# jcfaracco/xpysom-dask

Hardware: AMD Instinct MI355X
Metric: samples/sec/epoch (higher is better)
Workload: dtype f16

## Files before the change

### xpysom_dask_amd/_lib.py

```python
import ctypes as C
import importlib.util
import os

HERE = os.path.dirname(os.path.abspath(__file__))
LIB_PATH = os.environ.get("SOM_LIB_PATH") or os.path.join(HERE, "libsomhip.so")

SOM_DIST = {"euclidean": 0, "euclidean_no_opt": 1, "cosine": 2, "manhattan": 3, "manhattan_no_opt": 3,
            "norm_p": 4, "norm_p_no_opt": 5}
SOM_NEIGH = {"gaussian": 0, "mexican_hat": 1, "bubble": 2, "triangle": 3}
SOM_PREC = {"f32": 0, "bf16": 1, "f16": 3, "exact": 5}
SOM_TOPO = {"rectangular": 0, "hexagonal": 1}
SOM_BMU_ACTIVATION, SOM_BMU_QUANTIZATION = 0, 1
SOM_KERNELS = {"bmu": 0, "segsum": 1, "kron": 2, "merge": 3, "prep": 4, "screen": 5}


class SomConfig(C.Structure):
    _fields_ = [("x", C.c_int32), ("y", C.c_int32), ("input_len", C.c_int32),
                ("distance", C.c_int32), ("neighborhood", C.c_int32),
                ("compact_support", C.c_int32), ("precision", C.c_int32), ("device", C.c_int32),
                ("std_coeff", C.c_double), ("stream", C.c_void_p),
                ("topology", C.c_int32), ("norm_p", C.c_int32), ("norm_p_real", C.c_double)]


_F = C.POINTER(C.c_float)
# ... 28 lines not shown
    "som_pinned_free": (C.c_int, [C.c_void_p]),
    "som_stream_begin": (C.c_int, [_H]),
    "som_stream_rows": (C.c_int, [_H, _F, C.c_int64]),
    "som_stream_end": (C.c_int, [_H, C.c_double, C.c_double, C.c_int]),
    "som_accum_device_ptr": (C.c_int, [_H, C.POINTER(C.c_void_p), C.POINTER(C.c_int64)]),
    "som_get_stream": (C.c_int, [_H, C.POINTER(C.c_void_p)]),
    "som_epoch_fetch": (C.c_int, [_H, _F, _F, _I]),
    "som_epoch_accumulate_forced": (C.c_int, [_H, _I, C.c_double, C.c_double, C.c_int]),
    "som_bmu": (C.c_int, [_H, _F, C.c_int64, C.c_int32, _I]),
    "som_bmu_device": (C.c_int, [_H, C.c_void_p, C.c_int64, C.c_int32, _I]),
    "som_bmu_top2": (C.c_int, [_H, _F, C.c_int64, _I, _I]),
    "som_bmu_top2_device": (C.c_int, [_H, C.c_void_p, C.c_int64, _I, _I]),
    "som_bmu_f64": (C.c_int, [_H, C.POINTER(C.c_double), C.c_int64, _I]),
    "som_distance_matrix": (C.c_int, [_H, _F, C.c_int64, C.c_int32, _F]),
    "som_quantization_error": (C.c_int, [_H, _F, C.c_int64, C.POINTER(C.c_double)]),
    "som_quantization_error_device": (C.c_int, [_H, C.c_void_p, C.c_int64, C.POINTER(C.c_double)]),
    "som_set_verify": (C.c_int, [_H, C.c_int32]),
    "som_verify_stats": (C.c_int, [_H, C.POINTER(C.c_int64), C.POINTER(C.c_int64)]),
    "som_debug_corrupt_operands": (C.c_int, [_H, C.c_int32]),
    "som_debug_mfma16": (C.c_int, [_H, C.c_void_p, C.c_void_p, _F, _F, C.c_int32]),
    "som_debug_stamps": (C.c_int, [_H, C.c_int64, C.c_void_p]),
    "som_debug_device_bytes": (C.c_int, [C.POINTER(C.c_int64)]),
    "som_debug_qe_stats": (C.c_int, [_H, C.POINTER(C.c_int64), C.POINTER(C.c_int64)]),
    "som_policy_eval": (C.c_int, [C.c_int32, C.POINTER(C.c_double), C.POINTER(C.c_double), C.POINTER(C.c_int32)]),
    "som_policy_replay": (C.c_int, [C.c_int32, C.POINTER(C.c_double), C.POINTER(C.c_double)]),
    "som_patch_order": (C.c_int, [C.c_int32, C.c_int32, _I]),
    "som_exact_stats": (C.c_int, [_H, C.POINTER(C.c_int64), C.POINTER(C.c_int64), C.POINTER(C.c_int64)]),
    "som_exact_top2_stats": (C.c_int, [_H, C.POINTER(C.c_int64), C.POINTER(C.c_int64)]),
    "som_exact_skip_stats": (C.c_int, [_H, C.POINTER(C.c_int64), C.POINTER(C.c_int64)]),
    "som_exact_resident_stats": (C.c_int, [_H, C.POINTER(C.c_int64), C.POINTER(C.c_int64)]),
    "som_exact_scout_stats": (C.c_int, [_H, C.POINTER(C.c_int64), C.POINTER(C.c_int64)]),
    "som_exact_refine_stats": (C.c_int, [_H, C.POINTER(C.c_int64), C.POINTER(C.c_int64)]),
    "som_exact_last_counts": (C.c_int, [_H, _I, C.c_int64]),
    "som_sync": (C.c_int, [_H]),
    "som_profile_enable": (C.c_int, [_H, C.c_int32]),
    "som_profile_get": (C.c_int, [_H, C.c_int32, C.POINTER(C.c_double), C.POINTER(C.c_int64)]),
    "som_profile_reset": (C.c_int, [_H]),
}

_lib = None


def torch_lib_file(name):
    try:
        spec = importlib.util.find_spec("torch")
    except (ImportError, ValueError):
# ... 46 lines not shown
```

### xpysom_dask_amd/csrc/bmu_bf16_k16.hpp

```cpp
#pragma once
#include "bmu_bf16.hpp"

namespace somhip {

constexpr int K16_T = 4;
constexpr int K16_STAGE_UNITS = 16 * K16_T;
constexpr int K16_SB = 4;
constexpr int K16_NW = 4;
constexpr int K16_WG_SAMPLES = K16_NW * 16 * K16_SB;

__host__ __device__ constexpr int k16_stage_bytes(int ks32) { return (K16_T * ks32 + 1) * 1024; }

template <int KS32, class EL = Bf16>
__global__ __launch_bounds__(256) void prep_w_bf16_k16_kernel(const float* __restrict__ W, int K, int D,
                                                              char* __restrict__ Wst, int n_stages,
                                                              const float* __restrict__ unit_wsq,
                                                              const float* __restrict__ scale_max2 = nullptr) {
    using E = typename EL::T;
    using bf16x8 = typename V8<E>::t;
    long id = (long)blockIdx.x * 256 + threadIdx.x;
    long total = (long)n_stages * K16_T * KS32 * 64;
    if (id >= total) return;
    int lane = id & 63;
    long t = id >> 6;
    int ks = t % KS32; t /= KS32;
    int t16 = t % K16_T;
    long stage = t / K16_T;
    long u = stage * K16_STAGE_UNITS + t16 * 16 + (lane & 15);
    int k0 = ks * 32 + (lane >> 4) * 8;
    float scale = 1.0f;
    if (unit_wsq != nullptr && u < K) { float q = unit_wsq[u]; scale = q > 0.0f ? 1.0f / __builtin_sqrtf(q) : 0.0f; }
    if (scale_max2 != nullptr) scale = ex_scale(*scale_max2);
    bf16x8 v;
#pragma unroll
    for (int j = 0; j < 8; ++j) {
        float f = (u < K && k0 + j < D) ? W[u * D + k0 + j] * scale : 0.0f;
        v[j] = cvt<E>(-f);
    }
    *(bf16x8*)(Wst + stage * k16_stage_bytes(KS32) + ((long)(t16 * KS32 + ks) * 64 + lane) * 16) = v;
}

template <int KS32, class EL = Bf16>
__global__ __launch_bounds__(256) void prep_w_exact_k16_kernel(const float* __restrict__ W, int K, int D,
                                                               char* __restrict__ Wst, int n_stages,
                                                               const float* __restrict__ scale_max2,
                                                               float* __restrict__ werr2, char* __restrict__ Wst_lo = nullptr) {
    using E = typename EL::T;
    using bf16x8 = typename V8<E>::t;
    const int lane = threadIdx.x & 63;
    const long tile = (long)blockIdx.x * 4 + (threadIdx.x >> 6);
    if (tile >= (long)n_stages * K16_T) return;
    const long stage = tile / K16_T;
    const int t16 = (int)(tile - stage * K16_T);
    const long u = stage * K16_STAGE_UNITS + t16 * 16 + (lane & 15);
    const float scale = ex_scale(*scale_max2);
    float er = 0.0f;
#pragma unroll
    for (int ks = 0; ks < KS32; ++ks) {
        const int k0 = ks * 32 + (lane >> 4) * 8;
        bf16x8 v, vl;
#pragma unroll
        for (int j = 0; j < 8; ++j) {
            const float f = (u < K && k0 + j < D) ? W[u * D + k0 + j] * scale : 0.0f;
            const E hb = cvt<E>(-f);
            v[j] = hb;
            const float e = half_operand_error(-f, (float)hb);
            er = __builtin_fmaf(e, e, er);
            const float r = ((-f) - (float)hb) * 2048.0f;
            vl[j] = cvt<E>(r == r && __builtin_fabsf(r) < 3.0e38f ? r : 0.0f);
        }
        *(bf16x8*)(Wst + stage * k16_stage_bytes(KS32) + ((long)(t16 * KS32 + ks) * 64 + lane) * 16) = v;
        if (Wst_lo != nullptr) *(bf16x8*)(Wst_lo + stage * k16_stage_bytes(KS32) + ((long)(t16 * KS32 + ks) * 64 + lane) * 16) = vl;
    }
    er += __shfl_xor(er, 16, 64);
    er += __shfl_xor(er, 32, 64);
    float m = (er == er) ? er : 0.0f;
#pragma unroll
    for (int o = 8; o > 0; o >>= 1) m = fmaxf(m, __shfl_xor(m, o, 64));
    if (lane == 0) atomic_max_pos_f32(werr2, m);
}

constexpr int MP_TILES = 4;
template <int KS32, class EL = Bf16>
__global__ __launch_bounds__(64 * KS32) void merge_prep_k16_kernel(float* __restrict__ W, const float* __restrict__ ACC,
                                                                 int K, int D, int D1p, char* __restrict__ Wst,
                                                                 float* __restrict__ wn, float* __restrict__ wmax2,
                                                                 long n_tiles) {
    using E = typename EL::T;
    using bf16x8 = typename V8<E>::t;
    __shared__ float red[MP_TILES][KS32][16];
    const int lane = threadIdx.x & 63, ks = threadIdx.x >> 6;
    const int k0 = ks * 32 + (lane >> 4) * 8;
    const bool full = k0 + 8 <= D && (D & 3) == 0;
    float w[MP_TILES][8], den[MP_TILES];
    long unit[MP_TILES];
#pragma unroll
    for (int i = 0; i < MP_TILES; ++i) {
        const long tile = (long)blockIdx.x * MP_TILES + i;
        const long stage = tile / K16_T;
        const long u = stage * K16_STAGE_UNITS + (tile - stage * K16_T) * 16 + (lane & 15);
        unit[i] = (tile < n_tiles && u < K) ? u : -1;
        den[i] = 0.0f;
// ... 387 lines not shown
```

### xpysom_dask_amd/csrc/exact_host.hpp

```cpp

struct PassCtr {
    int* base; int n_groups;
    int* gcount() const { return base; }
    int* gstart() const { return base + n_groups; }
    PassCounters* tail() const { return (PassCounters*)(gstart() + n_groups); }
    RowNeed* row_need() const { return (RowNeed*)base; }
    size_t bytes() const { return 2 * (size_t)n_groups * sizeof(int) + sizeof(PassCounters); }
};
inline PassCtr pass_ctr(const som_handle* h) { return PassCtr{h->ex.ctr, (int)cdiv(h->K, EX_GROUP)}; }

constexpr double EX_KAPPA = 6.0;
ExactBound exact_bound(const som_handle* h) {
    const double u = std::ldexp(1.0, -24);
    const double Dl = h->wide ? 32.0 * h->ft_kchunks : 8.0 * h->fr_kg;
    const double n_mfma = h->wide ? h->n_kchunks : h->ks32;
    const double gamma = Dl * u / (1.0 - Dl * u);
    const double slop = 1.01;
    ExactBound eb{};
    eb.cB = (float)(slop * 2.0 * (EX_KAPPA * n_mfma + 1.0) * std::ldexp(1.0, -23));
    eb.cM = (float)(slop * 2.0);
    if (h->cfg.distance == SOM_DIST_COSINE) {
        eb.cA = (float)(slop * 2.0 * (gamma + 57.0 * u));
        eb.cW = 0.0f;
        eb.unit = 1;
// ... 176 lines not shown
    int* table = scratch + 4 * n;
    int* tot = table + 256L * B;
    const int passes = std::max(1, (int)cdiv(bits, 8));
    const int* kin = keys_in; const int* vin = nullptr;
    for (int p = 0; p < passes; ++p) {
        const bool last = p == passes - 1;
        int* ko = last ? keys_out : (p & 1) ? kb : ka;
        int* vo = last ? vals_out : (p & 1) ? vb : va;
        rs_hist_kernel<<<dim3((unsigned)B), dim3(256), 0, h->stream>>>(kin, n, 8 * p, B, table);
        rs_scan_kernel<<<dim3(64), dim3(256), 0, h->stream>>>(table, B, tot);
        rs_scatter_kernel<<<dim3((unsigned)B), dim3(256), 0, h->stream>>>(kin, vin, n, 8 * p, B, table, tot, ko, vo);
        kin = ko; vin = vo;
    }
    HIPCHK(h, hipGetLastError());
    return 0;
}

int exact_skip_reserve(som_handle* h, som_handle::ExactScratch::SortedRows& sr, long rows, long stride) {
    auto& ex = h->ex;
    if (ex.hook_refuse_skip) return fail(h, "exact: block-skipping scratch refused (test hook)");
    const long n_groups = cdiv(h->K, EX_GROUP);
    if (!ex.cen_ready) {
        for (auto& c : ex.cen) c = som_handle::ExactScratch::Centroids{};
        const int ncs = (int)cdiv(n_groups, K16_STAGE_UNITS);
        for (int lv = 0; lv < (h->wide ? 1 : 2); ++lv) {
            auto& c = ex.cen[lv];
            c.n_slots = lv == 0 ? (int)n_groups : (int)cdiv(n_groups, 4) * 16;
            c.n_cstages = lv == 0 ? ncs : 4 * ncs;
            c.n_img_stages = h->wide ? (int)cdiv(n_groups, WD_STAGE_UNITS) : c.n_cstages;
            if (int rc = c.Cc.alloc(h, (size_t)c.n_slots * h->D)) return rc;
            if (int rc = c.rg.alloc(h, (size_t)c.n_slots)) return rc;
            if (int rc = c.csq.alloc(h, (size_t)c.n_slots)) return rc;
            if (int rc = c.cmax2.alloc(h, 2)) return rc;
            if (int rc = c.Cst.alloc(h, (size_t)c.n_img_stages * h->stage_bytes)) return rc;
            HIPCHK(h, hipMemsetAsync(c.Cst, 0, (size_t)c.n_img_stages * h->stage_bytes, h->stream));
            if (lv == 0) {
                if (int rc = c.Cst_plain.alloc(h, (size_t)c.n_img_stages * h->stage_bytes)) return rc;
                HIPCHK(h, hipMemsetAsync(c.Cst_plain, 0, (size_t)c.n_img_stages * h->stage_bytes, h->stream));
            }
        }
        ex.cen_ready = true;
    }
    const long need_rows = round_up(rows, SK_TILE);
    if (need_rows > sr.cap) {
        HIPCHK(h, hipStreamSynchronize(h->stream));
        sr = som_handle::ExactScratch::SortedRows{};
// ... 22 lines not shown
        if (int rc = ex.tq.alloc(h, (size_t)stride)) return rc;
    if (int rc = ex.need.alloc(h, (size_t)tiles * ex.cen[0].n_cstages)) return rc;
    if (int rc = ex.need2.alloc(h, (size_t)tiles * ex.cen[1].n_cstages)) return rc;
    if (int rc = ex.glist.alloc(h, (size_t)tiles * n_groups)) return rc;
    if (int rc = ex.gcnt.alloc(h, (size_t)tiles)) return rc;
    if (int rc = ex.tile_counts.alloc(h, (size_t)tiles)) return rc;
    if (int rc = ex.tlist.alloc(h, (size_t)tiles * n_groups * K16_T)) return rc;
    if (int rc = ex.tcnt.alloc(h, (size_t)tiles)) return rc;
    ex.item_slots = (int)resident_slots(h, 8);
    if (int rc = ex.items.alloc(h, (size_t)(5 * tiles + 4 * ex.item_slots + 16))) return rc;
    if (int rc = ex.sk_tmp.alloc(h, radix_scratch_ints(stride))) return rc;
    ex.sk_stride = stride;
    return 0;
}

template <class E>
int exact_skip_centroids(som_handle* h, const float* xmax2) {
    auto& ex = h->ex;
    const float* Wsrc = h->ex_patch ? h->Wp : h->W;
    const int n_groups = (int)cdiv(h->K, EX_GROUP);
    auto& c0 = ex.cen[0];
    auto& c1 = ex.cen[1];
    const CentroidLevel l1{c0.Cc, c0.rg, c0.csq, c0.cmax2, c0.n_slots}, l2{c1.Cc, c1.rg, c1.csq, c1.cmax2, c1.n_slots};
    exact_centroids_kernel<<<dim3((unsigned)(cdiv(n_groups, 4) * 4)), dim3(512), 0, h->stream>>>(Wsrc, h->K, h->D, n_groups, l1, l2, h->wmax2);
    const int nst2 = ex.lp.level2 ? c1.n_cstages : 0;
    char* plain = ex.lp.scout ? c0.Cst_plain : nullptr;
    const dim3 tgrid((unsigned)cdiv((long)(c0.n_cstages + nst2) * K16_T, 4)), block(256);
    switch (h->ks32) {
#define SOM_CIMG_CASE(k) case k: exact_centroid_image_kernel<k, E><<<tgrid, block, 0, h->stream>>>(l1, c0.Cst, c0.n_cstages, l2, c1.Cst, nst2, h->D, xmax2, h->wmax2, plain); break;
    SOM_CIMG_CASE(1) SOM_CIMG_CASE(2) SOM_CIMG_CASE(3) SOM_CIMG_CASE(4)
#undef SOM_CIMG_CASE
    default: return fail(h, "exact: block skipping supports input_len <= 128");
    }
    HIPCHK(h, hipGetLastError());
    return 0;
}

int exact_skip_sortkeys(som_handle* h, som_handle::ExactScratch::SortedRows& sr, long s0, long n, const int* prev, const int* scout_g) {
    auto& ex = h->ex;
    const int n_groups = (int)cdiv(h->K, EX_GROUP);
    if (scout_g != nullptr)
        exact_groupkey_kernel<<<dim3((unsigned)cdiv(n, 256)), dim3(256), 0, h->stream>>>(scout_g, n, n_groups, ex.sk_keys, ex.sk_vals);
    else
        exact_sortkey_kernel<<<dim3((unsigned)cdiv(n, 256)), dim3(256), 0, h->stream>>>(prev, h->ex_inv, n, h->K, ex.sk_keys, ex.sk_vals);
    int bits = 1;
    while ((1L << bits) < n_groups) ++bits;
    return radix_sort_rows(h, ex.sk_keys, n, bits, ex.sk_keys2, sr.order + s0, ex.sk_tmp);
}
template <class E>
int exact_skip_gather(som_handle* h, som_handle::ExactScratch::SortedRows& sr, long s0, const int* order, const float* X, const __bf16* Xb, long n,
                      const float* xsq, const float* xerr, const float* xmax2) {
    const long np = round_up(n, SK_TILE);
    exact_gather_sorted_kernel<E><<<dim3((unsigned)cdiv(np, 16)), dim3(256), 0, h->stream>>>(
        order, n, np, h->dp, h->D, Xb, X, xsq, xerr, xmax2, sr.Xb_s + s0 * h->dp, sr.Xl_s != nullptr ? sr.Xl_s + s0 * h->dp : nullptr, sr.Xf_s + s0 * h->D,
        sr.xsq_s + s0, sr.xerr_s + s0);
    HIPCHK(h, hipGetLastError());
    return 0;
// ... 587 lines not shown
```

### xpysom_dask_amd/csrc/exact_skip.hpp

```cpp
#pragma once
#include "bmu_bf16_k16.hpp"

namespace somhip {

constexpr int SK_TILE = K16_WG_SAMPLES;
static_assert(K16_STAGE_UNITS == 64 && K16_T == 4, "block skipping: a stage of the resident screen is one 64-unit group of four 16-unit tiles");

struct CentroidLevel { float* C; float* rg; float* csq; float* cmax2; int n_slots; };
__global__ __launch_bounds__(512) void exact_centroids_kernel(const float* __restrict__ W, int K, int D, int n_groups,
                                                              CentroidLevel l1, CentroidLevel l2, const float* __restrict__ wmax2) {
    __shared__ float qsum[4][128];
    __shared__ float part[2][64][2];
    __shared__ float csq_s[2][5];
    const int g = blockIdx.x, tid = threadIdx.x, lane = tid & 63;
    const int d = tid & 127, q = tid >> 7, fh = (tid >> 6) & 1;
    const long u0 = (long)g * 64 + 16 * q;
    const int cnt = (int)max(0L, min(64L, (long)K - (long)g * 64));
    const int cb = max(0, min(16, cnt - 16 * q));
    if (g == 0 && tid == 0) { l1.cmax2[0] = *wmax2; l1.cmax2[1] = 0.0f; l2.cmax2[0] = *wmax2; l2.cmax2[1] = 0.0f; }
    float w[16];
#pragma unroll
    for (int k = 0; k < 16; ++k) w[k] = (d < D && k < cb) ? W[(u0 + k) * D + d] : 0.0f;
    float sum = 0.0f;
#pragma unroll
    for (int k = 0; k < 16; ++k) sum += w[k];
    qsum[q][d] = sum;
    __syncthreads();
    const float cs = cb > 0 ? sum / (float)cb : 0.0f;
    const float cg = cnt > 0 ? ((qsum[0][d] + qsum[1][d]) + (qsum[2][d] + qsum[3][d])) / (float)cnt : 0.0f;
    if (d < D) {
        if (q == 0 && g < l1.n_slots) l1.C[(long)g * D + d] = cg;
        const int j = 16 * (g >> 2) + 4 * (g & 3) + q;
        if (j < l2.n_slots) l2.C[(long)j * D + d] = cs;
    }
    {
        const float a = wave_sum(cs * cs);
        if (lane == 0) csq_s[fh][1 + q] = a;
        if (q == 0) { const float bq = wave_sum(cg * cg); if (lane == 0) csq_s[fh][0] = bq; }
    }
#pragma unroll
    for (int k = 0; k < 16; ++k) {
        if (k < cb) {
            const float dg = w[k] - cg, ds = w[k] - cs;
            const float qg = wave_sum(d < D ? dg * dg : 0.0f);
            const float qs = wave_sum(d < D ? ds * ds : 0.0f);
            if (lane == 0) { part[fh][16 * q + k][0] = qg; part[fh][16 * q + k][1] = qs; }
        }
    }
    __syncthreads();
    if (tid < 5) {
        const int b = tid - 1;
        const int k0 = tid == 0 ? 0 : 16 * b, k1 = tid == 0 ? cnt : min(cnt, 16 * b + 16);
        float m = 0.0f;
        for (int k = k0; k < k1; ++k) {
            const float d2 = part[0][k][tid == 0 ? 0 : 1] + part[1][k][tid == 0 ? 0 : 1];
            m = (d2 > m || !(d2 == d2)) ? d2 : m;
        }
        const float r = k1 > k0 ? __builtin_sqrtf(m) * (1.0f + 1.0f / 512.0f) + 1.0e-30f : -1.0f;
        const float sq = csq_s[0][tid] + csq_s[1][tid];
        if (tid == 0) { if (g < l1.n_slots) { l1.rg[g] = r; l1.csq[g] = sq; } }
        else {
            const int j = 16 * (g >> 2) + 4 * (g & 3) + b;
            if (j < l2.n_slots) { l2.rg[j] = r; l2.csq[j] = sq; }
        }
    }
}

__global__ __launch_bounds__(256) void exact_sortkey_kernel(const int* __restrict__ prev, const int* __restrict__ inv, long n,
                                                            int K, int* __restrict__ keys, int* __restrict__ vals) {
    const long i = (long)blockIdx.x * 256 + threadIdx.x;
    if (i >= n) return;
    int u = prev[i];
    u = u < 0 ? 0 : u >= K ? K - 1 : u;
    keys[i] = (inv != nullptr ? inv[u] : u) >> 6;
    vals[i] = (int)i;
}

__global__ __launch_bounds__(256) void exact_lastpos_kernel(const int* __restrict__ prev, const int* __restrict__ order,
                                                            const int* __restrict__ inv, long n, int K, int* __restrict__ lastpos) {
    const long p = (long)blockIdx.x * 256 + threadIdx.x;
    if (p >= n) return;
    int u = prev[order[p]];
    u = u < 0 ? 0 : u >= K ? K - 1 : u;
    lastpos[p] = inv != nullptr ? inv[u] : u;
}

template <class EL>
__global__ __launch_bounds__(256) void exact_gather_sorted_kernel(const int* __restrict__ order, long n, long np, int dp, int D,
// ... 647 lines not shown
```

### xpysom_dask_amd/csrc/somhip.hip

```cpp
#include <hip/hip_runtime.h>

#include <cstring>

#include <dlfcn.h>

#include <cmath>
#include <cstdio>
#include <cstdlib>
#include <algorithm>
#include <atomic>
#include <cstring>
#include <string>
#include <utility>
#include <vector>

#include "../../include/somhip.h"
#include "../../include/somhip_test.h"
#include "bmu_bf16_k16.hpp"
#include "bmu_bf16_tiled.hpp"
#include "bmu_bf16_wide.hpp"
#include "bmu_exact.hpp"
#include "exact_skip.hpp"
#include "exact_policy.hpp"
#include "exact_skip_wide.hpp"
#include "bmu_f32.hpp"
#include "bmu_f32_res.hpp"
#include "bmu_f32_tiled.hpp"
#include "bmu_pairwise.hpp"
#include "update.hpp"

using namespace somhip;

namespace {

thread_local std::string g_create_error;

const char* dev_env(const char* name) {
    static const bool on = [] { const char* v = std::getenv("SOM_TEST_HOOKS"); return v != nullptr && std::atoi(v) != 0; }();
    return on ? std::getenv(name) : nullptr;
}

struct EventPair { hipEvent_t a, b; int kernel; };

}

// ... 67 lines not shown
        DevBuf<float> fbX;
        PassCounters* pass_host = nullptr;
        hipEvent_t fb_ready = nullptr;
        int64_t rows_total = 0, rows_fallback = 0, chunks = 0;
        int64_t blocks_run = 0, blocks_total = 0;
        long pass_rows_override = 0;
        long hook_refuse_above = 0, hook_pairs = 0; bool hook_refuse_skip = false;
        long stride_cap = 0;
        long pairs = 64;
        int skip_mode = 1;
        policy::PlanState plan;
        policy::LaunchPlan lp;
        bool sub_blocks = true;
        struct SortedRows {
            long cap = 0;
            DevBuf<int> order;
            DevBuf<__bf16> Xb_s;
            DevBuf<__bf16> Xl_s;
            bool xl_filled = false;
            DevBuf<float> Xf_s, xsq_s, xerr_s, seed_s, sU_s;
            DevBuf<int> lastpos_s;
        } srt[2];
        bool cen_ready = false;
        long sk_stride = 0;
        int res_every = 0;
        DevBuf<int> sk_keys, sk_keys2, sk_vals;
        DevBuf<int> sk_tmp;
        bool refine_on = true;
        int grid_mult = 2;
        bool scout_on = true;
        DevBuf<int> scout_g;
        DevBuf<float> tq;
        double share_forecast = 1.0;
        struct Cost {
            hipEvent_t ev[8] = {};
            bool have = false;
        } cost;
        struct Centroids { DevBuf<float> Cc, rg, csq, cmax2; DevBuf<char> Cst;
                           DevBuf<char> Cst_plain;
                           int n_slots = 0, n_cstages = 0, n_img_stages = 0; } cen[2];
        DevBuf<unsigned long long> need, need2;
        DevBuf<int> glist, gcnt;
        DevBuf<int> tlist, tcnt;
        DevBuf<int2> tile_counts;
        DevBuf<int2> items;
        int item_slots = 0;
// ... 217 lines not shown
        float ms = 0.f;
        HIPCHK(h, hipEventElapsedTime(&ms, ep.a, ep.b));
        h->ms[ep.kernel] += ms;
        h->launches[ep.kernel] += 1;
        h->pool.push_back(ep);
    }
    h->pending.clear();
    return 0;
}

#define SOM_HALF(h, fn, ...) ((h)->f16 ? fn<F16>(__VA_ARGS__) : fn<Bf16>(__VA_ARGS__))
#define SOM_KS32_DISPATCH(fn, ...) \
    switch (h->ks32) { \
    case 1: return fn<1, E>(__VA_ARGS__); case 2: return fn<2, E>(__VA_ARGS__); case 3: return fn<3, E>(__VA_ARGS__); case 4: return fn<4, E>(__VA_ARGS__); }
#define SOM_WIDE_DISPATCH(fn, ...) \
    switch (h->n_kchunks) { \
    case 5: return fn<5, E>(__VA_ARGS__); case 6: return fn<6, E>(__VA_ARGS__); case 7: return fn<7, E>(__VA_ARGS__); case 8: return fn<8, E>(__VA_ARGS__); \
    case 9: return fn<9, E>(__VA_ARGS__); case 10: return fn<10, E>(__VA_ARGS__); case 11: return fn<11, E>(__VA_ARGS__); case 12: return fn<12, E>(__VA_ARGS__); \
    case 13: return fn<13, E>(__VA_ARGS__); case 14: return fn<14, E>(__VA_ARGS__); case 15: return fn<15, E>(__VA_ARGS__); case 16: return fn<16, E>(__VA_ARGS__); \
    case 17: return fn<17, E>(__VA_ARGS__); case 18: return fn<18, E>(__VA_ARGS__); case 19: return fn<19, E>(__VA_ARGS__); case 20: return fn<20, E>(__VA_ARGS__); \
    case 21: return fn<21, E>(__VA_ARGS__); case 22: return fn<22, E>(__VA_ARGS__); case 23: return fn<23, E>(__VA_ARGS__); case 24: return fn<24, E>(__VA_ARGS__); \
    case 25: return fn<25, E>(__VA_ARGS__); }

void mark_codebook_changed(som_handle* h) { h->w_dirty = h->wsq_dirty = h->wf_dirty = h->wp_dirty = true; }

template <class E>
int prep_codebook_half(som_handle* h) {
    const float* unit = h->cfg.distance == SOM_DIST_COSINE ? h->wsq : nullptr;
    const float* Wex = h->ex_patch ? h->Wp : h->W;
    const float* qex = h->ex_patch ? h->wsq_p : h->wsq;
    const dim3 block(256);
    if (h->tiled) {
        if (h->wide && h->exact) {
            if (unit) unit = qex;
            if (unit) {
                HIPCHK(h, hipMemsetAsync(h->wn, 0, (size_t)h->K * sizeof(float), h->stream));
                HIPCHK(h, hipMemsetD32Async((hipDeviceptr_t)h->wmax2, 0x3F800000, 1, h->stream));
            } else {
                HIPCHK(h, hipMemsetAsync(h->wmax2, 0, sizeof(float), h->stream));
                exact_copy_wsq_kernel<<<dim3((unsigned)cdiv(h->K, 1024)), dim3(1024), 0, h->stream>>>(qex, h->K, h->wn, h->wmax2);
            }
            long total = (long)h->n_stages * WD_T * h->n_kchunks * 64;
            prep_w_bf16_wide_kernel<E><<<dim3((unsigned)cdiv(total, 256)), block, 0, h->stream>>>(
                Wex, h->K, h->D, h->n_kchunks, h->Wst, h->n_stages, unit, h->wmax2);
            HIPCHK(h, hipMemsetAsync(h->wmax2 + 1, 0, sizeof(float), h->stream));
            exact_werr_kernel<E><<<dim3((unsigned)cdiv(h->K, 4 * EX_WERR_UNITS)), block, 0, h->stream>>>(Wex, h->K, h->D, h->wmax2, h->wmax2 + 1, unit);
            return 0;
// ... 1233 lines not shown
    return 0;
}

int som_stream_end(som_handle* h, double sigma, double eta, int neigh_f64) {
    DeviceGuard dev_guard(h);
    if (!h) return 1;
    if (!h->streaming) return fail(h, "som_stream_end: call som_stream_begin first");
    h->streaming = false;
    return run_transform(h, sigma, eta, neigh_f64);
}

int som_epoch_merge(som_handle* h) {
    DeviceGuard dev_guard(h);
    if (!h) return 1;
    Timed t(h, SOM_K_MERGE);
    if (h->fuse_merge_prep && ((is_half1(h) && !h->tiled && h->cfg.distance == SOM_DIST_EUCLIDEAN) ||
                               (h->wide && !h->exact && h->n_kchunks <= 4 * WD_MP_ITERS))) {
        if (int rc = SOM_HALF(h, merge_prep_half, h)) return rc;
        HIPCHK(h, hipGetLastError());
        mark_codebook_changed(h);
        h->w_dirty = false;
        return 0;
    }
    long total = (long)h->K * h->D;
    const bool keep_wp = h->ex_patch && !h->wp_dirty;
    merge_kernel<<<dim3((unsigned)cdiv(total, 256)), dim3(256), 0, h->stream>>>(h->W, h->ACC, h->K, h->D, h->D1p,
                                                                                keep_wp ? h->Wp : nullptr, h->ex_inv);
    HIPCHK(h, hipGetLastError());
    mark_codebook_changed(h);
    if (keep_wp) h->wp_dirty = false;
    return 0;
}

int som_epoch_accumulate_begin(som_handle* h, double sigma, double eta, int neigh_f64);
int som_epoch_accumulate_block(som_handle* h, int32_t block, int64_t* offset, int64_t* n_floats);

namespace {
int rccl_load(const char* path) {
    if (g_rccl.lib) return 0;
    const char* search[] = {"librccl.so", "librccl.so.1", "/opt/rocm/lib/librccl.so.1"};
    const char* only[] = {path};
    const char* const* cands = path ? only : search;
    const int n_cands = path ? 1 : 3;
    void* lib = nullptr;
    for (int i = 0; i < n_cands && !lib; ++i) lib = dlopen(cands[i], RTLD_NOW | RTLD_NOLOAD);
    std::string why;
// ... 426 lines not shown
    return 0;
}

int som_debug_mfma16(som_handle* h, const uint16_t* a_host, const uint16_t* b_host, const float* c_host, float* d_host,
                     int32_t is_f16) {
    DeviceGuard dev_guard(h);
    if (!h || !a_host || !b_host || !c_host || !d_host) return fail(h, "som_debug_mfma16: NULL argument");
    DevBuf<uint16_t> a, b;
    DevBuf<float> c, d;
    int rc = 0;
    if ((rc = a.alloc(h, 512)) || (rc = b.alloc(h, 512)) || (rc = c.alloc(h, 256)) || (rc = d.alloc(h, 256))) return rc;
    if (h2d_blocking(h, a, a_host, 1024) || h2d_blocking(h, b, b_host, 1024) || h2d_blocking(h, c, c_host, 1024)) return 1;
    if (is_f16) debug_mfma16_kernel<F16><<<dim3(1), dim3(64), 0, h->stream>>>(a, b, c, d);
    else debug_mfma16_kernel<Bf16><<<dim3(1), dim3(64), 0, h->stream>>>(a, b, c, d);
    return d2h_blocking(h, d_host, d, 1024);
}

int som_debug_device_bytes(int64_t* out) {
    if (!out) return 1;
    *out = g_dev_bytes.load();
    return 0;
}

int som_debug_qe_stats(som_handle* h, int64_t* rows, int64_t* rows_sqrt) {
    if (!h || !rows || !rows_sqrt) return fail(h, "som_debug_qe_stats: NULL argument");
    *rows = h->qe_rows;
    *rows_sqrt = h->qe_rows_sqrt;
    return 0;
}

int som_debug_stamps(som_handle* h, int64_t n_pairs, uint64_t* out_host) {
    DeviceGuard dev_guard(h);
    if (!h) return 1;
#ifdef SOM_STAMPS
    static unsigned long long* buf = nullptr;
    static int64_t cap = 0;
    HIPCHK(h, hipStreamSynchronize(h->stream));
    if (out_host) {
        if (n_pairs > cap) return fail(h, "som_debug_stamps: more pairs than the buffer holds");
        HIPCHK(h, hipMemcpy(out_host, buf, (size_t)n_pairs * 16, hipMemcpyDeviceToHost));
        return 0;
    }
    if (buf) { (void)hipFree(buf); buf = nullptr; cap = 0; }
    if (n_pairs > 0) {
        HIPCHK(h, hipMalloc((void**)&buf, (size_t)n_pairs * 16));
        HIPCHK(h, hipMemset(buf, 0, (size_t)n_pairs * 16));
// ... 98 lines not shown
```

### xpysom_dask_amd/engine.py

```python
import ctypes as C

import numpy as np

from . import _lib


class SomHipError(RuntimeError):
    pass


def _f32(a):
    return np.ascontiguousarray(a, dtype=np.float32)


class HipEngine:
    def __init__(self, x, y, input_len, *, distance="euclidean", neighborhood="gaussian",
                 std_coeff=0.5, compact_support=False, precision="exact", device=0, stream=None,
                 topology="rectangular", norm_p=0, norm_p_real=0.0):
        self._lib = _lib.load()
        self._h = None
        self.K, self.D = int(x) * int(y), int(input_len)
        self.x, self.y = int(x), int(y)
        self.n_rows = 0
        self._keepalive = None
# ... 239 lines not shown

    def debug_corrupt_operands(self, which=3):
        self._check(self._lib.som_debug_corrupt_operands(self._h, int(which)))

    def debug_mfma16(self, a, b, c, f16=True):
        a = np.ascontiguousarray(a).view(np.uint16).reshape(16, 32)
        b = np.ascontiguousarray(b).view(np.uint16).reshape(32, 16)
        c = np.ascontiguousarray(c, dtype=np.float32).reshape(16, 16)
        d = np.empty((16, 16), dtype=np.float32)
        self._check(self._lib.som_debug_mfma16(self._h, a.ctypes.data_as(C.c_void_p), b.ctypes.data_as(C.c_void_p),
                                               self._fp(c), self._fp(d), int(bool(f16))))
        return d

    def exact_stats(self):
        a, b, c = C.c_int64(), C.c_int64(), C.c_int64()
        self._check(self._lib.som_exact_stats(self._h, C.byref(a), C.byref(b), C.byref(c)))
        return a.value, b.value, c.value

    def qe_stats(self):
        a, b = C.c_int64(), C.c_int64()
        self._check(self._lib.som_debug_qe_stats(self._h, C.byref(a), C.byref(b)))
        return a.value, b.value

    def exact_top2_stats(self):
        a, b = C.c_int64(), C.c_int64()
        self._check(self._lib.som_exact_top2_stats(self._h, C.byref(a), C.byref(b)))
        return a.value, b.value

    def exact_skip_stats(self):
        a, b = C.c_int64(), C.c_int64()
        self._check(self._lib.som_exact_skip_stats(self._h, C.byref(a), C.byref(b)))
        return a.value, b.value

    def exact_resident_stats(self):
        a, b = C.c_int64(), C.c_int64()
        self._check(self._lib.som_exact_resident_stats(self._h, C.byref(a), C.byref(b)))
        return a.value, b.value

    def exact_scout_stats(self):
        a, b = C.c_int64(), C.c_int64()
        self._check(self._lib.som_exact_scout_stats(self._h, C.byref(a), C.byref(b)))
        return a.value, b.value

    def exact_refine_stats(self):
        a, b = C.c_int64(), C.c_int64()
        self._check(self._lib.som_exact_refine_stats(self._h, C.byref(a), C.byref(b)))
# ... 21 lines not shown
```

Before: 506.1 million.

## Fuse exact-mode merge with operand prep and centroid computation

Adds a fused merge path for exact precision. Two kernels replace the separate merge kernel and the later prep passes: the first divides accumulators, writes W/Wp, the squared norms, the f32 resident stage image and the centroids from shared memory, and the second builds the hi/lo half-precision stage images. A cen_current flag lets the screen skip relaunching the centroid kernel when the fused merge already produced the centroids. This removes several kernel launches and re-reads of the codebook per epoch, at the cost of more complex state tracking. It also adds a debug readback API.

```diff
diff --git a/xpysom_dask_amd/_lib.py b/xpysom_dask_amd/_lib.py
--- a/xpysom_dask_amd/_lib.py
+++ b/xpysom_dask_amd/_lib.py
@@ -74,6 +74,7 @@
     "som_debug_stamps": (C.c_int, [_H, C.c_int64, C.c_void_p]),
     "som_debug_device_bytes": (C.c_int, [C.POINTER(C.c_int64)]),
     "som_debug_qe_stats": (C.c_int, [_H, C.POINTER(C.c_int64), C.POINTER(C.c_int64)]),
+    "som_debug_read_operands": (C.c_int, [_H, C.c_int32, C.c_void_p, C.c_int64]),
     "som_policy_eval": (C.c_int, [C.c_int32, C.POINTER(C.c_double), C.POINTER(C.c_double), C.POINTER(C.c_int32)]),
     "som_policy_replay": (C.c_int, [C.c_int32, C.POINTER(C.c_double), C.POINTER(C.c_double)]),
     "som_patch_order": (C.c_int, [C.c_int32, C.c_int32, _I]),
diff --git a/xpysom_dask_amd/csrc/bmu_bf16_k16.hpp b/xpysom_dask_amd/csrc/bmu_bf16_k16.hpp
--- a/xpysom_dask_amd/csrc/bmu_bf16_k16.hpp
+++ b/xpysom_dask_amd/csrc/bmu_bf16_k16.hpp
@@ -40,6 +40,24 @@
     *(bf16x8*)(Wst + stage * k16_stage_bytes(KS32) + ((long)(t16 * KS32 + ks) * 64 + lane) * 16) = v;
 }
 
+template <class E>
+__device__ __forceinline__ void exact_operand_halves(float f, E& hi, E& lo, float& er) {
+    const E hb = cvt<E>(-f);
+    hi = hb;
+    const float e = half_operand_error(-f, (float)hb);
+    er = __builtin_fmaf(e, e, er);
+    const float r = ((-f) - (float)hb) * 2048.0f;
+    lo = cvt<E>(r == r && __builtin_fabsf(r) < 3.0e38f ? r : 0.0f);
+}
+__device__ __forceinline__ void exact_operand_error_max(float er, int lane, float* werr2) {
+    er += __shfl_xor(er, 16, 64);
+    er += __shfl_xor(er, 32, 64);
+    float m = (er == er) ? er : 0.0f;
+#pragma unroll
+    for (int o = 8; o > 0; o >>= 1) m = fmaxf(m, __shfl_xor(m, o, 64));
+    if (lane == 0) atomic_max_pos_f32(werr2, m);
+}
+
 template <int KS32, class EL = Bf16>
 __global__ __launch_bounds__(256) void prep_w_exact_k16_kernel(const float* __restrict__ W, int K, int D,
                                                                char* __restrict__ Wst, int n_stages,
@@ -62,22 +80,15 @@
 #pragma unroll
         for (int j = 0; j < 8; ++j) {
             const float f = (u < K && k0 + j < D) ? W[u * D + k0 + j] * scale : 0.0f;
-            const E hb = cvt<E>(-f);
-            v[j] = hb;
-            const float e = half_operand_error(-f, (float)hb);
-            er = __builtin_fmaf(e, e, er);
-            const float r = ((-f) - (float)hb) * 2048.0f;
-            vl[j] = cvt<E>(r == r && __builtin_fabsf(r) < 3.0e38f ? r : 0.0f);
+            E hi, lo;
+            exact_operand_halves<E>(f, hi, lo, er);
+            v[j] = hi;
+            vl[j] = lo;
         }
         *(bf16x8*)(Wst + stage * k16_stage_bytes(KS32) + ((long)(t16 * KS32 + ks) * 64 + lane) * 16) = v;
         if (Wst_lo != nullptr) *(bf16x8*)(Wst_lo + stage * k16_stage_bytes(KS32) + ((long)(t16 * KS32 + ks) * 64 + lane) * 16) = vl;
     }
-    er += __shfl_xor(er, 16, 64);
-    er += __shfl_xor(er, 32, 64);
-    float m = (er == er) ? er : 0.0f;
-#pragma unroll
-    for (int o = 8; o > 0; o >>= 1) m = fmaxf(m, __shfl_xor(m, o, 64));
-    if (lane == 0) atomic_max_pos_f32(werr2, m);
+    exact_operand_error_max(er, lane, werr2);
 }
 
 constexpr int MP_TILES = 4;
diff --git a/xpysom_dask_amd/csrc/exact_host.hpp b/xpysom_dask_amd/csrc/exact_host.hpp
--- a/xpysom_dask_amd/csrc/exact_host.hpp
+++ b/xpysom_dask_amd/csrc/exact_host.hpp
@@ -222,6 +222,7 @@
     const long n_groups = cdiv(h->K, EX_GROUP);
     if (!ex.cen_ready) {
         for (auto& c : ex.cen) c = som_handle::ExactScratch::Centroids{};
+        ex.cen_current = false;
         const int ncs = (int)cdiv(n_groups, K16_STAGE_UNITS);
         for (int lv = 0; lv < (h->wide ? 1 : 2); ++lv) {
             auto& c = ex.cen[lv];
@@ -290,7 +291,11 @@
     auto& c0 = ex.cen[0];
     auto& c1 = ex.cen[1];
     const CentroidLevel l1{c0.Cc, c0.rg, c0.csq, c0.cmax2, c0.n_slots}, l2{c1.Cc, c1.rg, c1.csq, c1.cmax2, c1.n_slots};
-    exact_centroids_kernel<<<dim3((unsigned)(cdiv(n_groups, 4) * 4)), dim3(512), 0, h->stream>>>(Wsrc, h->K, h->D, n_groups, l1, l2, h->wmax2);
+    if (!ex.cen_current) {
+        exact_centroids_kernel<<<dim3((unsigned)(cdiv(n_groups, 4) * 4)), dim3(512), 0, h->stream>>>(Wsrc, h->K, h->D, n_groups, l1, l2, h->wmax2);
+        ++ex.centroid_launches;
+        ex.cen_current = h->fuse_merge_prep;
+    }
     const int nst2 = ex.lp.level2 ? c1.n_cstages : 0;
     char* plain = ex.lp.scout ? c0.Cst_plain : nullptr;
     const dim3 tgrid((unsigned)cdiv((long)(c0.n_cstages + nst2) * K16_T, 4)), block(256);
@@ -301,6 +306,38 @@
     default: return fail(h, "exact: block skipping supports input_len <= 128");
     }
     HIPCHK(h, hipGetLastError());
+    return 0;
+}
+
+template <class E>
+int merge_exact_operands(som_handle* h) {
+    auto& ex = h->ex;
+    const int n_groups = (int)cdiv(h->K, EX_GROUP);
+    const bool cen = ex.cen_ready;
+    auto& c0 = ex.cen[0];
+    auto& c1 = ex.cen[1];
+    CentroidLevel l1{}, l2{};
+    if (cen) {
+        l1 = CentroidLevel{c0.Cc, c0.rg, c0.csq, c0.cmax2, c0.n_slots};
+        l2 = CentroidLevel{c1.Cc, c1.rg, c1.csq, c1.cmax2, c1.n_slots};
+    }
+    HIPCHK(h, hipMemsetAsync(h->wmax2, 0, 2 * sizeof(float), h->stream));
+    const dim3 agrid((unsigned)(cen ? cdiv(n_groups, 4) * 4 : n_groups)), bgrid((unsigned)h->n_stages);
+    float* Wp = h->ex_patch ? (float*)h->Wp : nullptr;
+    float* wsq_p = h->ex_patch ? (float*)h->wsq_p : nullptr;
+    const int* perm = h->ex_patch ? (const int*)h->ex_perm : nullptr;
+    const float* Wsrc = h->ex_patch ? h->Wp : h->W;
+    switch (h->ks32) {
+#define SOM_MX_CASE(k) case k: \
+        merge_exact_a_kernel<k><<<agrid, dim3(512), 0, h->stream>>>(h->ACC, perm, h->K, h->D, h->D1p, n_groups, h->fr_kg, h->W, Wp, h->wsq, wsq_p, \
+                                                                   h->wn, h->wmax2, h->Wfst, cen ? 1 : 0, l1, l2); \
+        merge_exact_b_kernel<k, E><<<bgrid, dim3(256), 0, h->stream>>>(Wsrc, h->K, h->D, h->Wst, h->Wst_lo, h->wmax2, h->wmax2 + 1, \
+                                                                      cen ? (float*)c0.cmax2 : nullptr, cen ? (float*)c1.cmax2 : nullptr); \
+        break;
+    SOM_MX_CASE(1) SOM_MX_CASE(2) SOM_MX_CASE(3) SOM_MX_CASE(4)
+#undef SOM_MX_CASE
+    default: return fail(h, "exact: the fused merge supports input_len <= 128");
+    }
     return 0;
 }
 
diff --git a/xpysom_dask_amd/csrc/exact_skip.hpp b/xpysom_dask_amd/csrc/exact_skip.hpp
--- a/xpysom_dask_amd/csrc/exact_skip.hpp
+++ b/xpysom_dask_amd/csrc/exact_skip.hpp
@@ -7,20 +7,15 @@
 static_assert(K16_STAGE_UNITS == 64 && K16_T == 4, "block skipping: a stage of the resident screen is one 64-unit group of four 16-unit tiles");
 
 struct CentroidLevel { float* C; float* rg; float* csq; float* cmax2; int n_slots; };
-__global__ __launch_bounds__(512) void exact_centroids_kernel(const float* __restrict__ W, int K, int D, int n_groups,
-                                                              CentroidLevel l1, CentroidLevel l2, const float* __restrict__ wmax2) {
+__device__ __forceinline__ void exact_centroids_group(const float (&w)[16], int g, int K, int D, const CentroidLevel& l1,
+                                                      const CentroidLevel& l2) {
     __shared__ float qsum[4][128];
     __shared__ float part[2][64][2];
     __shared__ float csq_s[2][5];
-    const int g = blockIdx.x, tid = threadIdx.x, lane = tid & 63;
+    const int tid = threadIdx.x, lane = tid & 63;
     const int d = tid & 127, q = tid >> 7, fh = (tid >> 6) & 1;
-    const long u0 = (long)g * 64 + 16 * q;
     const int cnt = (int)max(0L, min(64L, (long)K - (long)g * 64));
     const int cb = max(0, min(16, cnt - 16 * q));
-    if (g == 0 && tid == 0) { l1.cmax2[0] = *wmax2; l1.cmax2[1] = 0.0f; l2.cmax2[0] = *wmax2; l2.cmax2[1] = 0.0f; }
-    float w[16];
-#pragma unroll
-    for (int k = 0; k < 16; ++k) w[k] = (d < D && k < cb) ? W[(u0 + k) * D + d] : 0.0f;
     float sum = 0.0f;
 #pragma unroll
     for (int k = 0; k < 16; ++k) sum += w[k];
@@ -64,6 +59,20 @@
             if (j < l2.n_slots) { l2.rg[j] = r; l2.csq[j] = sq; }
         }
     }
+}
+
+__global__ __launch_bounds__(512) void exact_centroids_kernel(const float* __restrict__ W, int K, int D, int n_groups,
+                                                              CentroidLevel l1, CentroidLevel l2, const float* __restrict__ wmax2) {
+    const int g = blockIdx.x, tid = threadIdx.x;
+    const int d = tid & 127, q = tid >> 7;
+    const long u0 = (long)g * 64 + 16 * q;
+    const int cnt = (int)max(0L, min(64L, (long)K - (long)g * 64));
+    const int cb = max(0, min(16, cnt - 16 * q));
+    if (g == 0 && tid == 0) { l1.cmax2[0] = *wmax2; l1.cmax2[1] = 0.0f; l2.cmax2[0] = *wmax2; l2.cmax2[1] = 0.0f; }
+    float w[16];
+#pragma unroll
+    for (int k = 0; k < 16; ++k) w[k] = (d < D && k < cb) ? W[(u0 + k) * D + d] : 0.0f;
+    exact_centroids_group(w, g, K, D, l1, l2);
 }
 
 __global__ __launch_bounds__(256) void exact_sortkey_kernel(const int* __restrict__ prev, const int* __restrict__ inv, long n,
diff --git a/xpysom_dask_amd/csrc/merge_exact.hpp b/xpysom_dask_amd/csrc/merge_exact.hpp
--- /dev/null
+++ b/xpysom_dask_amd/csrc/merge_exact.hpp
@@ -0,0 +1,189 @@
+#pragma once
+#include "bmu_exact.hpp"
+#include "bmu_f32_res.hpp"
+#include "exact_skip.hpp"
+
+namespace somhip {
+
+static_assert(EX_GROUP == 64 && FR_STAGE_UNITS == 64 && K16_STAGE_UNITS == 64, "merge_exact: one group = one stage of both images");
+
+__host__ __device__ constexpr int mx_stride(int D) { return D | 1; }
+
+template <int KS32>
+__global__ __launch_bounds__(512) void merge_exact_a_kernel(const float* __restrict__ ACC, const int* __restrict__ perm, int K, int D,
+                                                            int D1p, int n_groups, int kg, float* __restrict__ W,
+                                                            float* __restrict__ Wp, float* __restrict__ wsq, float* __restrict__ wsq_p,
+                                                            float* __restrict__ wn, float* __restrict__ wmax2, char* __restrict__ Wfst,
+                                                            int centroids, CentroidLevel l1, CentroidLevel l2) {
+    constexpr int DMAX = 32 * KS32;
+    __shared__ float rows[64 * mx_stride(DMAX)];
+    __shared__ int unit_s[64];
+    __shared__ float den_s[64];
+    const int g = blockIdx.x, tid = threadIdx.x;
+    const int S = mx_stride(D);
+    const long p0 = (long)g * 64;
+    if (tid < 64) {
+        const long pos = p0 + tid;
+        const int u = pos < K ? (perm != nullptr ? perm[pos] : (int)pos) : -1;
+        unit_s[tid] = u;
+        den_s[tid] = u >= 0 ? ACC[(long)u * D1p + D] : 0.0f;
+    }
+    __syncthreads();
+    if (g < n_groups) {
+        if ((D & 3) == 0) {
+            const int q4 = D >> 2, total = 64 * q4;
+            f32x4 a[KS32];
+#pragma unroll
+            for (int it = 0; it < KS32; ++it) {
+                const int i = tid + 512 * it;
+                a[it] = f32x4{0.0f, 0.0f, 0.0f, 0.0f};
+                if (i < total) {
+                    const int r = i / q4, c = i - r * q4, u = unit_s[r];
+                    if (u >= 0)
+                        a[it] = den_s[r] != 0.0f ? *(const f32x4*)(ACC + (long)u * D1p + 4 * c) : *(const f32x4*)(W + (long)u * D + 4 * c);
+                }
+            }
+#pragma unroll
+            for (int it = 0; it < KS32; ++it) {
+                const int i = tid + 512 * it;
+                if (i >= total) continue;
+                const int r = i / q4, c = i - r * q4, u = unit_s[r];
+                if (u < 0) continue;
+                const float den = den_s[r];
+                f32x4 v = a[it];
+                if (den != 0.0f) {
+#pragma unroll
+                    for (int j = 0; j < 4; ++j) v[j] = v[j] / den;
+                    *(f32x4*)(W + (long)u * D + 4 * c) = v;
+                }
+                if (Wp != nullptr) *(f32x4*)(Wp + (p0 + r) * D + 4 * c) = v;
+#pragma unroll
+                for (int j = 0; j < 4; ++j) rows[r * S + 4 * c + j] = v[j];
+            }
+        } else {
+            const int total = 64 * D;
+#pragma unroll
+            for (int it = 0; it < 4 * KS32; ++it) {
+                const int i = tid + 512 * it;
+                if (i >= total) continue;
+                const int r = i / D, d = i - r * D, u = unit_s[r];
+                if (u < 0) continue;
+                const float den = den_s[r];
+                float v;
+                if (den != 0.0f) { v = ACC[(long)u * D1p + d] / den; W[(long)u * D + d] = v; }
+                else v = W[(long)u * D + d];
+                if (Wp != nullptr) Wp[(p0 + r) * D + d] = v;
+                rows[r * S + d] = v;
+            }
+        }
+    }
+    __syncthreads();
+    if (g < n_groups) {
+        char* stage = Wfst + (long)g * fr_stage_bytes(kg);
+        if (tid < 64) {
+            const int u = unit_s[tid];
+            float q = 0.0f;
+            if (u >= 0) {
+                q = np_pairwise_sq_sum(rows + tid * S, D);
+                wsq[u] = q;
+                if (wsq_p != nullptr) wsq_p[p0 + tid] = q;
+                wn[p0 + tid] = q;
+            }
+            ((float*)(stage + (long)FR_UT * kg * 1024))[tid] = u >= 0 ? q : __builtin_inff();
+            float m = (q == q) ? q : 0.0f;
+#pragma unroll
+            for (int o = 32; o > 0; o >>= 1) m = fmaxf(m, __shfl_xor(m, o, 64));
+            if (tid == 0) atomic_max_pos_f32(wmax2, m);
+        }
+        for (int r = tid; r < FR_UT * kg * 64; r += 512) {
+            const int lane = r & 63, t = r >> 6;
+            const int fg = t % kg, ut = t / kg;
+            const int row = ut * 32 + (lane & 31);
+            const bool live = unit_s[row] >= 0;
+            f32x4 v;
+#pragma unroll
+            for (int j = 0; j < 4; ++j) {
+                const int k = 8 * fg + 2 * j + (lane >> 5);
+                v[j] = (live && k < D) ? rows[row * S + k] : 0.0f;
+            }
+            *(f32x4*)(stage + ((long)(ut * kg + fg) * 64 + lane) * 16) = v;
+        }
+    }
+    if (centroids) {
+        const int d = tid & 127, q = tid >> 7;
+        const int cnt = (int)max(0L, min(64L, (long)K - p0));
+        const int cb = max(0, min(16, cnt - 16 * q));
+        float w[16];
+#pragma unroll
+        for (int k = 0; k < 16; ++k) w[k] = (d < D && k < cb) ? rows[(16 * q + k) * S + d] : 0.0f;
+        exact_centroids_group(w, g, K, D, l1, l2);
+    }
+}
+
+template <int KS32, class EL = Bf16>
+__global__ __launch_bounds__(256) void merge_exact_b_kernel(const float* __restrict__ Wsrc, int K, int D, char* __restrict__ Wst,
+                                                            char* __restrict__ Wst_lo, const float* __restrict__ scale_max2,
+                                                            float* __restrict__ werr2, float* __restrict__ cmax2_1,
+                                                            float* __restrict__ cmax2_2) {
+    using E = typename EL::T;
+    using bf16x8 = typename V8<E>::t;
+    constexpr int DMAX = 32 * KS32;
+    __shared__ float rows[64 * mx_stride(DMAX)];
+    const int tid = threadIdx.x, lane = tid & 63, t16 = tid >> 6;
+    const long stage = blockIdx.x;
+    const int S = mx_stride(D);
+    const int cnt = (int)min(64L, (long)K - stage * 64);
+    const float* src = Wsrc + stage * 64 * D;
+    if (blockIdx.x == 0 && tid == 0 && cmax2_1 != nullptr) {
+        cmax2_1[0] = *scale_max2; cmax2_1[1] = 0.0f; cmax2_2[0] = *scale_max2; cmax2_2[1] = 0.0f;
+    }
+    if ((D & 3) == 0) {
+        const int total = cnt * (D >> 2);
+        f32x4 a[2 * KS32];
+#pragma unroll
+        for (int it = 0; it < 2 * KS32; ++it) {
+            const int i = tid + 256 * it;
+            a[it] = i < total ? *(const f32x4*)(src + 4 * i) : f32x4{0.0f, 0.0f, 0.0f, 0.0f};
+        }
+#pragma unroll
+        for (int it = 0; it < 2 * KS32; ++it) {
+            const int i = tid + 256 * it;
+            if (i >= total) continue;
+            const int r = (4 * i) / D, c = 4 * i - r * D;
+#pragma unroll
+            for (int j = 0; j < 4; ++j) rows[r * S + c + j] = a[it][j];
+        }
+    } else {
+        const int total = cnt * D;
+#pragma unroll
+        for (int it = 0; it < 8 * KS32; ++it) {
+            const int i = tid + 256 * it;
+            if (i >= total) continue;
+            const int r = i / D;
+            rows[r * S + (i - r * D)] = src[i];
+        }
+    }
+    __syncthreads();
+    const int row = t16 * 16 + (lane & 15);
+    const long u = stage * K16_STAGE_UNITS + row;
+    const float scale = ex_scale(*scale_max2);
+    float er = 0.0f;
+#pragma unroll
+    for (int ks = 0; ks < KS32; ++ks) {
+        const int k0 = ks * 32 + (lane >> 4) * 8;
+        bf16x8 v, vl;
+#pragma unroll
+        for (int j = 0; j < 8; ++j) {
+            const float f = (u < K && k0 + j < D) ? rows[row * S + k0 + j] * scale : 0.0f;
+            E hi, lo;
+            exact_operand_halves<E>(f, hi, lo, er);
+            v[j] = hi;
+            vl[j] = lo;
+        }
+        *(bf16x8*)(Wst + stage * k16_stage_bytes(KS32) + ((long)(t16 * KS32 + ks) * 64 + lane) * 16) = v;
+        *(bf16x8*)(Wst_lo + stage * k16_stage_bytes(KS32) + ((long)(t16 * KS32 + ks) * 64 + lane) * 16) = vl;
+    }
+    exact_operand_error_max(er, lane, werr2);
+}
+
+}
diff --git a/xpysom_dask_amd/csrc/somhip.hip b/xpysom_dask_amd/csrc/somhip.hip
--- a/xpysom_dask_amd/csrc/somhip.hip
+++ b/xpysom_dask_amd/csrc/somhip.hip
@@ -21,6 +21,7 @@
 #include "bmu_bf16_wide.hpp"
 #include "bmu_exact.hpp"
 #include "exact_skip.hpp"
+#include "merge_exact.hpp"
 #include "exact_policy.hpp"
 #include "exact_skip_wide.hpp"
 #include "bmu_f32.hpp"
@@ -134,6 +135,8 @@
             DevBuf<int> lastpos_s;
         } srt[2];
         bool cen_ready = false;
+        bool cen_current = false;
+        int64_t centroid_launches = 0;
         long sk_stride = 0;
         int res_every = 0;
         DevBuf<int> sk_keys, sk_keys2, sk_vals;
@@ -397,7 +400,10 @@
     case 21: return fn<21, E>(__VA_ARGS__); case 22: return fn<22, E>(__VA_ARGS__); case 23: return fn<23, E>(__VA_ARGS__); case 24: return fn<24, E>(__VA_ARGS__); \
     case 25: return fn<25, E>(__VA_ARGS__); }
 
-void mark_codebook_changed(som_handle* h) { h->w_dirty = h->wsq_dirty = h->wf_dirty = h->wp_dirty = true; }
+void mark_codebook_changed(som_handle* h) {
+    h->w_dirty = h->wsq_dirty = h->wf_dirty = h->wp_dirty = true;
+    h->ex.cen_current = false;
+}
 
 template <class E>
 int prep_codebook_half(som_handle* h) {
@@ -1677,6 +1683,15 @@
         h->w_dirty = false;
         return 0;
     }
+    if (h->fuse_merge_prep && h->exact && !h->tiled) {
+        if (int rc = SOM_HALF(h, merge_exact_operands, h)) return rc;
+        HIPCHK(h, hipGetLastError());
+        mark_codebook_changed(h);
+        h->w_dirty = h->wsq_dirty = h->wf_dirty = h->wp_dirty = false;
+        h->wf_patch = h->ex_patch;
+        h->ex.cen_current = h->ex.cen_ready;
+        return 0;
+    }
     long total = (long)h->K * h->D;
     const bool keep_wp = h->ex_patch && !h->wp_dirty;
     merge_kernel<<<dim3((unsigned)cdiv(total, 256)), dim3(256), 0, h->stream>>>(h->W, h->ACC, h->K, h->D, h->D1p,
@@ -2149,6 +2164,43 @@
     return 0;
 }
 
+int som_debug_read_operands(som_handle* h, int32_t which, void* out_host, int64_t bytes) {
+    DeviceGuard dev_guard(h);
+    if (!h || !out_host) return fail(h, "som_debug_read_operands: NULL argument");
+    if (which == 14) {
+        if (bytes != (int64_t)sizeof(int64_t)) return fail(h, "som_debug_read_operands: wrong size");
+        *(int64_t*)out_host = h->ex.centroid_launches;
+        return 0;
+    }
+    const auto& c0 = h->ex.cen[0];
+    const auto& c1 = h->ex.cen[1];
+    const bool cen = h->ex.cen_ready && !h->wide;
+    const size_t K = (size_t)h->K, D = (size_t)h->D, f = sizeof(float);
+    const size_t img = (size_t)h->n_stages * h->stage_bytes;
+    const void* p = nullptr;
+    size_t n = 0;
+    switch (which) {
+    case 0: p = h->Wp; n = K * D * f; break;
+    case 1: p = h->wsq; n = K * f; break;
+    case 2: p = h->wsq_p; n = K * f; break;
+    case 3: p = h->wn; n = K * f; break;
+    case 4: p = h->wmax2; n = 2 * f; break;
+    case 5: p = h->Wfst; n = (size_t)h->fr_stages * fr_stage_bytes(h->fr_kg); break;
+    case 6: p = h->Wst; n = img; break;
+    case 7: p = h->Wst_lo; n = img; break;
+    case 8: if (cen) { p = c0.Cc; n = (size_t)c0.n_slots * D * f; } break;
+    case 9: if (cen) { p = c0.rg; n = (size_t)c0.n_slots * f; } break;
+    case 10: if (cen) { p = c0.csq; n = (size_t)c0.n_slots * f; } break;
+    case 11: if (cen) { p = c1.Cc; n = (size_t)c1.n_slots * D * f; } break;
+    case 12: if (cen) { p = c1.rg; n = (size_t)c1.n_slots * f; } break;
+    case 13: if (cen) { p = c1.csq; n = (size_t)c1.n_slots * f; } break;
+    default: return fail(h, "som_debug_read_operands: unknown buffer");
+    }
+    if (p == nullptr) return fail(h, "som_debug_read_operands: no such buffer on this handle");
+    if (bytes < 0 || (size_t)bytes != n) return fail(h, "som_debug_read_operands: wrong size");
+    return d2h_blocking(h, out_host, p, n);
+}
+
 int som_debug_qe_stats(som_handle* h, int64_t* rows, int64_t* rows_sqrt) {
     if (!h || !rows || !rows_sqrt) return fail(h, "som_debug_qe_stats: NULL argument");
     *rows = h->qe_rows;
diff --git a/xpysom_dask_amd/engine.py b/xpysom_dask_amd/engine.py
--- a/xpysom_dask_amd/engine.py
+++ b/xpysom_dask_amd/engine.py
@@ -285,6 +285,30 @@
         self._check(self._lib.som_debug_qe_stats(self._h, C.byref(a), C.byref(b)))
         return a.value, b.value
 
+    OPERANDS = ("Wp", "wsq", "wsq_p", "wn", "wmax2", "Wfst", "Wst", "Wst_lo", "Cc1", "rg1", "csq1", "Cc2", "rg2", "csq2")
+
+    def debug_read_operand(self, name):
+        K, D = self.K, self.D
+        groups = -(-K // 64)
+        ks32, kg = -(-D // 32), 1
+        while kg * 8 < D:
+            kg *= 2
+        img = groups * (4 * ks32 + 1) * 1024
+        slots = {"1": groups, "2": -(-groups // 4) * 16}
+        nbytes = {"Wp": 4 * K * D, "wsq": 4 * K, "wsq_p": 4 * K, "wn": 4 * K, "wmax2": 8, "Wfst": groups * (2 * kg + 1) * 1024,
+                  "Wst": img, "Wst_lo": img}
+        for lv, n in slots.items():
+            nbytes.update({"Cc" + lv: 4 * n * D, "rg" + lv: 4 * n, "csq" + lv: 4 * n})
+        out = np.empty(nbytes[name], dtype=np.uint8)
+        if self._lib.som_debug_read_operands(self._h, self.OPERANDS.index(name), out.ctypes.data_as(C.c_void_p), out.nbytes) != 0:
+            return None
+        return out if name in ("Wfst", "Wst", "Wst_lo") else out.view(np.float32)
+
+    def debug_centroid_launches(self):
+        n = C.c_int64()
+        self._check(self._lib.som_debug_read_operands(self._h, len(self.OPERANDS), C.byref(n), 8))
+        return n.value
+
     def exact_top2_stats(self):
         a, b = C.c_int64(), C.c_int64()
         self._check(self._lib.som_exact_top2_stats(self._h, C.byref(a), C.byref(b)))
```

After: 512.2 million, median of 6. 1.2% higher.
